# bcosm/CantorRL

Hardware: AMD Instinct MI355X
Metric: env-steps/sec (batched episodes) (higher is better)
Workload: dtype f64+f32; 1 GPU; configs[1]: 65,536 parallel envs/GPU, European call (BS rolling-ATM marks), GBM, v2 env, train_ppo_v2 reward; config_index=2, envs_per_gpu=65536, episode_length=252, mode=rollout, rollout_k=256, action_sets=1, parallelism=env-shard x1

## Files before the change

### cantorrl_amd/_lib.py

```python
import ctypes
import os

HERE = os.path.dirname(os.path.abspath(__file__))
LIB_PATH = os.environ.get("CANTORRL_HEDGEENV_LIB") or os.path.join(HERE, "lib", "libhedgeenv.so")

HE_ABI_VERSION = 4
HE_BOOK_MAX = 8
HE_OBS_DIM = 13
BOOK_TYPES = {"call": 0, "put": 1, "uo_call": 2}
HE_OK, HE_EINVAL, HE_ESHAPE, HE_EHIP, HE_ENOMEM, HE_ESTATE = range(6)
HE_MODE_REPLAY, HE_MODE_GBM, HE_MODE_HESTON = range(3)
HE_LOSS_MSE, HE_LOSS_ABS, HE_LOSS_CVAR, HE_LOSS_OTHER = range(4)
MODES = {"replay": HE_MODE_REPLAY, "gbm": HE_MODE_GBM, "heston": HE_MODE_HESTON}
HE_MARK_ROLLING_ATM, HE_MARK_FIXED_EUROPEAN = range(2)
MARKS = {"rolling_atm": HE_MARK_ROLLING_ATM, "fixed_european": HE_MARK_FIXED_EUROPEAN}


def loss_code(loss_type):
    return {"mse": HE_LOSS_MSE, "abs": HE_LOSS_ABS, "cvar": HE_LOSS_CVAR}.get(loss_type, HE_LOSS_OTHER)


class HeBookOption(ctypes.Structure):
    _fields_ = [
        ("type", ctypes.c_int32),
# ... 54 lines not shown
                            ("per_share_pnl_sum", "<f8"), ("reserved2", "<f8")])
assert EPISODE_RECORD.itemsize == 80

_P = ctypes.c_void_p
INFO_FIELDS = [
    ("step_pnl_total", "f8"), ("per_share_step_pnl", "f8"), ("raw_pnl_deviation_abs", "f8"),
    ("transaction_costs_total", "f8"), ("commission_cost", "f8"), ("slippage_cost", "f8"),
    ("reward_pnl_component", "f8"), ("transaction_cost_penalty", "f8"), ("theta_penalty", "f8"),
    ("reward_step", "f8"), ("portfolio_value", "f8"), ("cash", "f8"),
    ("call_contracts", "i4"), ("put_contracts", "i4"),
    ("scaled_float_call", "f4"), ("scaled_float_put", "f4"),
    ("requested_calls_rounded_clipped", "i4"), ("requested_puts_rounded_clipped", "i4"),
    ("actual_calls_traded", "i4"), ("actual_puts_traded", "i4"),
    ("initial_S0_for_episode", "f4"),
    ("current_stock_price", "f4"), ("current_volatility", "f4"),
    ("current_call_price", "f4"), ("current_put_price", "f4"), ("current_step", "i4"),
    ("current_episode_idx", "i4"),
]


class HeInfo(ctypes.Structure):
    _fields_ = [(name, _P) for name, _ in INFO_FIELDS]


EXPORTS = [
    "he_config_init", "he_create", "he_destroy", "he_last_error", "he_version", "he_load_paths",
    "he_seed", "he_reset", "he_reset_episodes", "he_step", "he_rollout", "he_num_envs", "he_episode_length",
    "he_num_episodes", "he_get_config", "he_state_size", "he_get_state", "he_set_state",
    "he_pcg64_seed_state", "he_host_episode_draws", "he_host_philox", "he_host_div_by", "he_host_div_byf", "he_time_next_step", "he_rollout_policy", "he_host_box_muller",
    "he_sync_market", "he_vecnorm_stats_len", "he_vecnorm_scratch_bytes", "he_vecnorm_init", "he_vecnorm_step",
    "he_vecnorm_apply", "he_vecnorm_attach", "he_vecnorm_attach_eval", "he_vecnorm_reset", "he_fixed_european_marks", "he_bs_delta_hedge", "he_count_nonfinite",
    "he_device_rng", "he_device_math", "he_host_math", "he_episode_summaries", "he_host_alloc", "he_host_free",
    "he_stream_wait", "he_step_signal", "he_signal_seq", "he_signal_wait", "he_host_episode_wrap",
    "he_host_vecnorm_sb3",
]


class HeVecnormParams(ctypes.Structure):
    _fields_ = [
        ("obs_dim", ctypes.c_int32),
        ("training", ctypes.c_int32),
        ("norm_obs", ctypes.c_int32),
        ("norm_reward", ctypes.c_int32),
        ("gamma", ctypes.c_double),
        ("clip_obs", ctypes.c_double),
        ("clip_reward", ctypes.c_double),
        ("epsilon", ctypes.c_double),
        ("moments", ctypes.c_int32),
        ("reserved", ctypes.c_int32 * 3),
    ]


HE_VN_MOMENTS_F64, HE_VN_MOMENTS_SB3 = range(2)
HE_VN_SB3_MAX_ENVS = 4096
VN_MOMENTS = {"f64": HE_VN_MOMENTS_F64, "sb3": HE_VN_MOMENTS_SB3}


class HeVecnormOut(ctypes.Structure):
    _fields_ = [(name, ctypes.c_void_p) for name in (
        "stats", "returns", "obs_out", "reward_out", "terminal_obs_out", "ep_return", "ep_length", "ep_return_done",
        "ep_length_done")]

_lib = None


class HedgeEnvError(RuntimeError):
    pass
# ... 26 lines not shown
        "he_step": (i32, [vp, vp, vp, vp, vp, vp, vp, ctypes.POINTER(HeInfo), vp]),
        "he_rollout": (i32, [vp, i32, vp, vp, vp, vp, vp]),
        "he_rollout_policy": (i32, [vp, i32, i32, vp, vp, vp, vp, vp, i64, vp, vp]),
        "he_num_envs": (i64, [vp]),
        "he_episode_length": (i32, [vp]),
        "he_num_episodes": (i64, [vp]),
        "he_get_config": (i32, [vp, ctypes.POINTER(HeConfig)]),
        "he_state_size": (ctypes.c_size_t, [vp]),
        "he_get_state": (i32, [vp, vp, ctypes.c_size_t]),
        "he_set_state": (i32, [vp, vp, ctypes.c_size_t]),
        "he_pcg64_seed_state": (i32, [u64, ctypes.POINTER(ctypes.c_uint64 * 4)]),
        "he_host_episode_draws": (i32, [u64, u64, i64, vp]),
        "he_host_philox": (i32, [u64, u64, u64, ctypes.POINTER(ctypes.c_uint32 * 4)]),
        "he_host_div_by": (i32, [ctypes.c_void_p, i64, ctypes.c_double, ctypes.c_void_p]),
        "he_host_div_byf": (i32, [ctypes.c_void_p, i64, ctypes.c_float, ctypes.c_void_p]),
        "he_host_box_muller": (i32, [ctypes.c_void_p, ctypes.c_void_p, i64, ctypes.c_void_p, ctypes.c_void_p]),
        "he_time_next_step": (i32, [vp, vp, vp]),
        "he_sync_market": (i32, [vp, vp]),
        "he_vecnorm_stats_len": (i64, [i32]),
        "he_vecnorm_scratch_bytes": (i64, [i64, i32]),
        "he_vecnorm_init": (i32, [vp, i32, vp]),
        "he_vecnorm_step": (i32, [ctypes.POINTER(HeVecnormParams), i64] + [vp] * 15 + [vp]),
        "he_vecnorm_apply": (i32, [ctypes.POINTER(HeVecnormParams), i64] + [vp] * 15 + [vp]),
        "he_vecnorm_attach": (i32, [vp, ctypes.POINTER(HeVecnormParams), vp, vp, vp]),
        "he_vecnorm_attach_eval": (i32, [vp, ctypes.POINTER(HeVecnormParams), ctypes.POINTER(HeVecnormOut)]),
        "he_vecnorm_reset": (i32, [ctypes.POINTER(HeVecnormParams), i64] + [vp] * 5 + [vp]),
        "he_host_vecnorm_sb3": (i32, [ctypes.POINTER(HeVecnormParams), i64] + [vp] * 9),
        "he_fixed_european_marks": (i32, [vp, i64, i32, ctypes.c_double, vp, vp, vp, vp]),
        "he_bs_delta_hedge": (i32, [vp, i64, i32, ctypes.c_double, ctypes.c_double, vp, vp]),
        "he_count_nonfinite": (i32, [vp, i64, vp, vp]),
        "he_device_rng": (i32, [u64, vp, vp, i64, vp, vp, vp]),
        "he_device_math": (i32, [i32, vp, i64, vp, vp]),
        "he_host_math": (i32, [i32, vp, i64, vp]),
        "he_host_episode_wrap": (i32, [vp, vp, vp, i64, i32, vp]),
        "he_episode_summaries": (i32, [vp, vp, vp]),
        "he_host_alloc": (i32, [ctypes.c_size_t, ctypes.POINTER(vp), ctypes.POINTER(vp)]),
        "he_host_free": (i32, [vp]),
        "he_stream_wait": (i32, [vp]),
        "he_step_signal": (i32, [vp, vp]),
        "he_signal_seq": (ctypes.c_uint32, [vp]),
        "he_signal_wait": (i32, [vp, vp, vp]),
    }
    ab = path != os.path.join(HERE, "lib", "libhedgeenv.so")
    for name, (res, args) in sig.items():
        if ab and not hasattr(lib, name):
            continue
        fn = getattr(lib, name)
        fn.restype = res
        fn.argtypes = args
    _lib = lib
    return lib


def check(lib, handle, status, what):
    if status != HE_OK:
        msg = lib.he_last_error(handle).decode() if handle else ""
        if status == HE_ESHAPE:
            raise ValueError(msg or "Data shapes are inconsistent.")
        raise HedgeEnvError(f"{what} failed (status {status}): {msg}")


def pcg64_seed_state(seed):
    lib = load()
    arr = (ctypes.c_uint64 * 4)()
    check(lib, None, lib.he_pcg64_seed_state(ctypes.c_uint64(seed), ctypes.byref(arr)), "he_pcg64_seed_state")
    return tuple(arr)
# ... 46 lines not shown
```

### cantorrl_amd/csrc/he_math.h

```cpp
#pragma once

#include <hip/hip_runtime.h>
#include <stdint.h>

#define HE_HD __host__ __device__ __forceinline__

namespace he {

HE_HD double fma_k(double a, double b, double c) {
#if defined(__HIP_DEVICE_COMPILE__)
    double r;
    asm("v_fma_f64 %0, %1, %2, %3" : "=v"(r) : "v"(a), "v"(b), "s"(c));
    return r;
#else
    return fma(a, b, c);
#endif
}

HE_HD double fma_kb(double a, double k, double c) {
#if defined(__HIP_DEVICE_COMPILE__)
    double r;
    asm("v_fma_f64 %0, %1, %2, %3" : "=v"(r) : "v"(a), "s"(k), "v"(c));
    return r;
#else
// ... 140 lines not shown
    return k <= T ? episode_wrap_le(t, k, T) : (t + k) % T;
}

struct u32x4 { uint32_t x, y, z, w; };

HE_HD uint32_t mulhi32(uint32_t a, uint32_t b) {
#if defined(__HIP_DEVICE_COMPILE__)
    return __umulhi(a, b);
#else
    return (uint32_t)(((uint64_t)a * (uint64_t)b) >> 32);
#endif
}

HE_HD u32x4 philox4x32_10(u32x4 c, uint32_t k0, uint32_t k1) {
    const uint32_t M0 = 0xD2511F53u, M1 = 0xCD9E8D57u;
    const uint32_t W0 = 0x9E3779B9u, W1 = 0xBB67AE85u;
#pragma unroll
    for (int r = 0; r < 10; ++r) {
        if (r) { k0 += W0; k1 += W1; }
        const uint64_t p0 = (uint64_t)M0 * c.x, p1 = (uint64_t)M1 * c.z;
        uint32_t hi0 = (uint32_t)(p0 >> 32), lo0 = (uint32_t)p0;
        uint32_t hi1 = (uint32_t)(p1 >> 32), lo1 = (uint32_t)p1;
        u32x4 o;
        o.x = hi1 ^ c.y ^ k0;
        o.y = lo1;
        o.z = hi0 ^ c.w ^ k1;
        o.w = lo0;
        c = o;
    }
    return c;
}

HE_HD double u01(uint32_t hi, uint32_t lo) {
    uint64_t k = ((((uint64_t)hi) << 32) | (uint64_t)lo) >> 12;
    return ((double)k + 0.5) * 2.220446049250313e-16;
}

HE_HD void sincos_2pi_u(double u2, double* sin_out, double* cos_out) {
    const double x = 4.0 * u2;
    const double q = rint(x);
    const double r = x - q;
    const double rr = r * r;
    double sp = 6.066935731106192e-12;
    sp = fma_k(sp, rr, -6.688035109811464e-10);
    sp = fma_k(sp, rr, 5.692172921967924e-08);
    sp = fma_k(sp, rr, -3.598843235212084e-06);
    sp = fma_k(sp, rr, 0.00016044118478735975);
    sp = fma_k(sp, rr, -0.004681754135318687);
    sp = fma_k(sp, rr, 0.07969262624616703);
    sp = fma_k(sp, rr, -0.6459640975062462);
    sp = fma_k(sp, rr, 1.5707963267948966);
    const double sn = r * sp;
    double cp = 6.565963114979468e-11;
    cp = fma_k(cp, rr, -6.386603083791849e-09);
    cp = fma_k(cp, rr, 4.710874778818169e-07);
    cp = fma_k(cp, rr, -2.5202042373060596e-05);
    cp = fma_k(cp, rr, 0.0009192602748394263);
    cp = fma_k(cp, rr, -0.020863480763352957);
    cp = fma_k(cp, rr, 0.253669507901048);
    cp = fma_k(cp, rr, -1.2337005501361697);
    const double cs = fma_k(cp, rr, 1.0);
    const int qi = (int)q & 3;
    const bool swp = (qi & 1) != 0;
    const double s_ = swp ? cs : sn, c_ = swp ? sn : cs;
    *sin_out = (qi & 2) ? -s_ : s_;
    *cos_out = ((qi + 1) & 2) ? -c_ : c_;
}

// ... 85 lines not shown
    p = fma_k(p, z, 0.005223977625442187842111847);
    p = fma_k(p, z, -0.02686617064513125175943235);
    p = fma_k(p, z, 0.1128379167095512573896159);
    p = fma_k(p, z, -0.376126389031837524632053);
    p = fma_k(p, z, 1.128379167095512573896159);
    return x * p;
}

HE_HD double ndtr(double a) {
    if (a != a) return a;
    const double SQRT1_2 = 0.70710678118654752440;
    double x = a * SQRT1_2;
    double z = fabs(x);
    double y;
    if (z < SQRT1_2) {
        y = 0.5 + 0.5 * erf_small(x);
    } else {
        y = 0.5 * erfc(z);
        if (x > 0) y = 1.0 - y;
    }
    return y;
}

HE_HD void ndtr_pair(double a, double* pos, double* neg) {
    if (a != a) {
        *pos = *neg = a;
        return;
    }
    const double SQRT1_2 = 0.70710678118654752440;
    double x = a * SQRT1_2;
    double z = fabs(x);
    if (z < SQRT1_2) {
        double e = (z < 0.25) ? erf_small4(x) : erf_small(x);
        *pos = 0.5 + 0.5 * e;
        *neg = 0.5 + 0.5 * (-e);
    } else {
        double y = 0.5 * erfc(z);
        if (x > 0) {
            *pos = 1.0 - y;
            *neg = y;
        } else {
            *pos = y;
            *neg = 1.0 - y;
        }
    }
}

HE_HD double norm_pdf(double x) {
    return exp(-(x * x) * 0.5) * 0.3989422804014327;
}

HE_HD double log_ratio(double S, double K) {
#if defined(__HIP_DEVICE_COMPILE__)
    double r = __builtin_amdgcn_rcp(K);
    r = fma(fma(-K, r, 1.0), r, r);
    r = fma(fma(-K, r, 1.0), r, r);
    const double y = (S - K) * r;
    if (!(fabs(y) < 0.0078125)) return log(S / K);
#else
    const double q = S / K;
    const double y = q - 1.0;
    if (!(fabs(y) < 0.0078125)) return log(q);
#endif
    double p = 1.0 / 9.0;
    p = fma_k(p, y, -1.0 / 8.0);
    p = fma_k(p, y, 1.0 / 7.0);
    p = fma_k(p, y, -1.0 / 6.0);
    p = fma_k(p, y, 1.0 / 5.0);
// ... 63 lines not shown
    for (int h = 0; h < NN; ++h) {
        const double xs = (fabs(x[h]) < 700.0) ? x[h] : 0.0;
        k[h] = rint(xs * 1.4426950408889634074);
        const double rh = fma_kb(-k[h], 6.93147180369123816490e-01, xs);
        r[h] = fma_kb(-k[h], 1.90821492927058770002e-10, rh);
        q[h] = 1.0 / 355687428096000.0;
    }
    constexpr double C[16] = {1.0 / 20922789888000.0, 1.0 / 1307674368000.0, 1.0 / 87178291200.0,
                              1.0 / 6227020800.0,     1.0 / 479001600.0,     1.0 / 39916800.0,
                              1.0 / 3628800.0,        1.0 / 362880.0,        1.0 / 40320.0,
                              1.0 / 5040.0,           1.0 / 720.0,           1.0 / 120.0,
                              1.0 / 24.0,             1.0 / 6.0,             0.5,
                              0.0};
#pragma unroll
    for (int c = 0; c < 15; ++c)
#pragma unroll
        for (int h = 0; h < NN; ++h) q[h] = fma_k(q[h], r[h], C[c]);
#pragma unroll
    for (int h = 0; h < NN; ++h) {
        const double s1 = 1.0 + r[h];
        const double e1 = (1.0 - s1) + r[h];
        out[h] = ldexp(s1 + fma(r[h] * r[h], q[h], e1), (int)k[h]);
    }
    bool big = false;
#pragma unroll
    for (int h = 0; h < NN; ++h) big = big || !(fabs(x[h]) < 700.0);
    if (he_any_lane(big)) {
#pragma unroll
        for (int h = 0; h < NN; ++h) out[h] = (fabs(x[h]) < 700.0) ? out[h] : exp(x[h]);
    }
}

template <int NN>
HE_HD void philox4x32_10_n(u32x4* c, uint32_t k0, uint32_t k1) {
    const uint32_t M0 = 0xD2511F53u, M1 = 0xCD9E8D57u;
    const uint32_t W0 = 0x9E3779B9u, W1 = 0xBB67AE85u;
#pragma unroll
    for (int rd = 0; rd < 10; ++rd) {
        if (rd) { k0 += W0; k1 += W1; }
#pragma unroll
        for (int h = 0; h < NN; ++h) {
            const uint64_t p0 = (uint64_t)M0 * c[h].x, p1 = (uint64_t)M1 * c[h].z;
            u32x4 o;
            o.x = (uint32_t)(p1 >> 32) ^ c[h].y ^ k0;
            o.y = (uint32_t)p1;
            o.z = (uint32_t)(p0 >> 32) ^ c[h].w ^ k1;
            o.w = (uint32_t)p0;
            c[h] = o;
        }
    }
}

template <int NN>
HE_HD void box_muller_n(const double* u1, const double* u2, double* z1, double* z2) {
    double s[NN], s2[NN], p[NN], ed[NN];
#pragma unroll
    for (int h = 0; h < NN; ++h) {
        int e;
        double m = frexp(u1[h], &e);
        const bool lo = m < 0.70710678118654752;
        m = lo ? m + m : m;
        ed[h] = (double)(lo ? e - 1 : e);
        s[h] = bm_quot(m);
        s2[h] = s[h] * s[h];
        p[h] = 1.0 / 19.0;
    }
// ... 41 lines not shown
        z1[h] = rad[h] * cosv;
        z2[h] = rad[h] * sinv;
    }
}

template <int NN>
HE_HD void ndtr_pair_n(const double* a, double* pos, double* neg) {
    const double SQRT1_2 = 0.70710678118654752440;
    double x[NN], z[NN], p[NN];
    bool easy = true;
#pragma unroll
    for (int h = 0; h < NN; ++h) {
        x[h] = a[h] * SQRT1_2;
        easy = easy && (fabs(x[h]) < 0.25);
        z[h] = x[h] * x[h];
        p[h] = 0.000001646211436588924740161296;
    }
    if (he_any_lane(!easy)) {
#pragma unroll
        for (int h = 0; h < NN; ++h) ndtr_pair(a[h], pos + h, neg + h);
        return;
    }
    constexpr double E[8] = {-0.00001492565035840625097746242, 0.0001205533298178966425102734,
                             -0.0008548327023450852832546658,  0.005223977625442187842111847,
                             -0.02686617064513125175943235,    0.1128379167095512573896159,
                             -0.376126389031837524632053,      1.128379167095512573896159};
#pragma unroll
    for (int c = 0; c < 8; ++c)
#pragma unroll
        for (int h = 0; h < NN; ++h) p[h] = fma_k(p[h], z[h], E[c]);
#pragma unroll
    for (int h = 0; h < NN; ++h) {
        const double e = x[h] * p[h];
        pos[h] = 0.5 + 0.5 * e;
        neg[h] = 0.5 + 0.5 * (-e);
    }
}

template <int NN>
HE_HD void log_ratio_n(const double* S, const double* K, double* out) {
    double y[NN], p[NN];
    bool easy = true;
#pragma unroll
    for (int h = 0; h < NN; ++h) {
#if defined(__HIP_DEVICE_COMPILE__)
        double r = __builtin_amdgcn_rcp(K[h]);
        r = fma(fma(-K[h], r, 1.0), r, r);
        r = fma(fma(-K[h], r, 1.0), r, r);
        y[h] = (S[h] - K[h]) * r;
#else
        const double q = S[h] / K[h];
        y[h] = q - 1.0;
#endif
        easy = easy && (fabs(y[h]) < 0.0078125);
        p[h] = 1.0 / 9.0;
    }
    if (he_any_lane(!easy)) {
#pragma unroll
        for (int h = 0; h < NN; ++h) out[h] = log_ratio(S[h], K[h]);
        return;
    }
    constexpr double L[8] = {-1.0 / 8.0, 1.0 / 7.0, -1.0 / 6.0, 1.0 / 5.0, -1.0 / 4.0, 1.0 / 3.0, -0.5, 1.0};
#pragma unroll
    for (int c = 0; c < 8; ++c)
#pragma unroll
        for (int h = 0; h < NN; ++h) p[h] = fma_k(p[h], y[h], L[c]);
#pragma unroll
    for (int h = 0; h < NN; ++h) out[h] = y[h] * p[h];
}

template <int NN>
HE_HD void bs_call_put_n(const double* S, const double* K, const BSConst& c, double* call, double* put) {
    if (c.intrinsic) {
#pragma unroll
        for (int h = 0; h < NN; ++h) bs_call_put(S[h], K[h], c, call + h, put + h);
        return;
    }
    double lr[NN], d[2 * NN], nd[2 * NN], md[2 * NN];
    log_ratio_n<NN>(S, K, lr);
#pragma unroll
    for (int h = 0; h < NN; ++h) {
        d[h] = (lr[h] + c.a) * c.inv_b;
        d[NN + h] = d[h] - c.b;
    }
    ndtr_pair_n<NN>(d, nd, md);
    ndtr_pair_n<NN>(d + NN, nd + NN, md + NN);
#pragma unroll
    for (int h = 0; h < NN; ++h) {
        const double Kd = K[h] * c.disc;
        const double cv = S[h] * nd[h] - Kd * nd[NN + h];
        const double pv = Kd * md[NN + h] - S[h] * md[h];
        call[h] = (cv < 0.0) ? 0.0 : cv;
        put[h] = (pv < 0.0) ? 0.0 : pv;
    }
}

struct Pcg64 {
    uint64_t sh, sl, ih, il;
    uint32_t has32, buf32;
};

HE_HD void pcg64_step(Pcg64& g) {
    const uint64_t MH = 0x2360ED051FC65DA4ull, ML = 0x4385DF649FCCF645ull;
#if defined(__HIP_DEVICE_COMPILE__)
    uint64_t lo = g.sl * ML;
    uint64_t hi = __umul64hi(g.sl, ML) + g.sl * MH + g.sh * ML;
#else
    unsigned __int128 p = (unsigned __int128)g.sl * ML;
    uint64_t lo = (uint64_t)p;
    uint64_t hi = (uint64_t)(p >> 64) + g.sl * MH + g.sh * ML;
#endif
    uint64_t nl = lo + g.il;
    uint64_t carry = nl < lo ? 1ull : 0ull;
    g.sl = nl;
    g.sh = hi + g.ih + carry;
}

HE_HD uint64_t pcg64_next64(Pcg64& g) {
    pcg64_step(g);
    uint64_t x = g.sh ^ g.sl;
    unsigned rot = (unsigned)(g.sh >> 58);
    return (x >> rot) | (x << ((64u - rot) & 63u));
}

HE_HD uint32_t pcg64_next32(Pcg64& g) {
    if (g.has32) {
// ... 50 lines not shown
```

### cantorrl_amd/csrc/hedge_env.hip

```cpp
#include <hip/hip_runtime.h>
#include <hip/hip_ext.h>

#include <math.h>
#include <stdarg.h>
#include <stdio.h>
#include <stdlib.h>
#include <string.h>

#include <chrono>
#include <new>
#include <type_traits>

#include "vn_moments.h"
#include <string>
#include <vector>

#include "../../include/hedge_env.h"
#include "he_math.h"

using namespace he;

namespace {

#define GLOBAL __attribute__((address_space(1)))
// ... 46 lines not shown
    double lnK, lnH, lnH2K;
    double invK;
    double invH;
};

struct Params {
    int64_t n;
    int64_t goff;
    int32_t T;
    int32_t variant, loss, record_metrics, autoreset, mode;
    int32_t tile_greeks;
    int32_t mt, maxh;
    float mt_f, maxh_f, T_f;
    float inv_maxh_f, inv_T_f;
    int32_t s0s_const;
    float s0s_f, inv_s0s_f;
    double s0s_d, inv_s0s_d;
    double inv_252;
    float init_cash_f;
    double tcpc, slip_frac, lam, w, theta, initial_cash;
    double shares_d, inv_shares;
    float shares_f;
    int32_t shares_zero;
    float r_f, tenor_f;
    double r_d, tenor_d, sqrt_tenor;
    int32_t tenor_small;
    uint32_t key0, key1;
    double s0;
    double var;
    float var_f;
    double sqrt_var, drift, sqrt_dt, mu, dt;
    BSConst bs;
    int32_t mark;
    double fe_K;
    float g_sigma, g_num_drift;
    double g_sst;
    double g_inv_sst;
    float g_sst_f, g_inv_sst_f;
    int32_t lds_tame;
    float sqrt_tenor_f;
    double h_kappa, h_theta, h_xi, h_rho, h_sqrt1mrho2;
    int32_t den_const;
    double den, inv_den;
    int32_t M;
    float4* tileA;
    float4* tileB;
    float rstv[4 + kObs];
    const float4* rec;
    const float4* recg;
    int64_t n_paths;
    int64_t rstride;
    int32_t roff;
    int32_t book_n;
    const BookOpt* book;
    const double* book_tab;
    int32_t book_rows;
    double bk_sig, bk_isig, bk_s2, bk_lam;
    double book_rst;
    double* tileC;
#ifdef HE_TIMING
    uint64_t* tim;
#endif
};

constexpr int32_t kRowOff = 7;
__host__ __device__ __forceinline__ int64_t replay_stride(int64_t T) { return ((T + 1 + kRowOff + 7) / 8) * 8; }
// ... 2189 lines not shown

            const int64_t gid = p.goff + pi;
            const uint64_t nf = a0 + (uint64_t)(kb + sl0);
            const uint32_t tpf = PLAIN ? 0u : episode_wrap(tpb, (uint32_t)sl0, T);
            double ex[kLdsH];
            double Vx[kLdsH];
            double Vin = Vbs;
            if constexpr (LOCK) {
                const uint64_t m0 = nf >> 1;
                const bool odd = (nf & 1) != 0;
                double zs[kLdsH];
                if (__ballot(odd) == 0ull) {
                    double zz[kLdsH];
                    philox_normals_n<kLdsH / 2>(p, gid, m0, zz);
#pragma unroll
                    for (int h = 0; h < kLdsH; ++h) zs[h] = zz[h];
                } else {
                    double zz[kLdsH + 2];
                    philox_normals_n<kLdsH / 2 + 1>(p, gid, m0, zz);
#pragma unroll
                    for (int h = 0; h < kLdsH; ++h) {
                        double a = zz[h], b = zz[h + 1];
                        asm volatile("" : "+v"(a), "+v"(b));
                        zs[h] = odd ? b : a;
                    }
                }
                double arg[kLdsH];
#pragma unroll
                for (int h = 0; h < kLdsH; ++h) {
                    Vx[h] = 0.0;
                    const double dW = p.sqrt_dt * zs[h];
                    arg[h] = p.drift + p.sqrt_var * dW;
                }
                exp_k_n<kLdsH>(arg, ex);
            } else if constexpr (!HESTON) {
                double zc = 0.0;
#pragma unroll
                for (int h = 0; h < kLdsH; ++h) {
                    ex[h] = 1.0;
                    Vx[h] = 0.0;
                    if (FULL || sl0 + h < len) {
                        const uint64_t n = nf + (uint64_t)h;
                        double z;
                        if (h == 0 || (n & 1) == 0) {
                            double z1, z2;
                            normals(p, gid, n >> 1, &z1, &z2);
                            z = (n & 1) ? z2 : z1;
                            zc = z2;
                        } else {
                            z = zc;
                        }
                        const double dW = p.sqrt_dt * z;
                        ex[h] = exp_k(p.drift + p.sqrt_var * dW);
                    }
                }
            } else {
                double w1[kLdsH], ws[kLdsH];
#pragma unroll
                for (int h = 0; h < kLdsH; ++h) w1[h] = ws[h] = 0.0;
#pragma unroll 1
                for (int h = 0; h < kLdsH; ++h) {
                    double a = 0.0, b = 0.0;
                    if (FULL || sl0 + h < len) {
                        double z1, z2;
                        normals(p, gid, nf + (uint64_t)h, &z1, &z2);
                        const double dw1 = p.sqrt_dt * z1, dw2 = p.sqrt_dt * z2;
                        a = dw1;
// ... 24 lines not shown
                    if (FULL || j < len) {
                        if (tq == 0) v = p.var;
                        vp = v < 0.0 ? 0.0 : v;
                        sq = sqrt(vp);
                        v = (v + p.h_kappa * (p.h_theta - vp) * p.dt) + p.h_xi * sq * w1all[j];
                        tq = (tq + 1 == T) ? 0u : tq + 1;
                    }
#pragma unroll
                    for (int h = 0; h < kLdsH; ++h) {
                        vpx[h] = (j == sl0 + h) ? vp : vpx[h];
                        sqx[h] = (j == sl0 + h) ? sq : sqx[h];
                        Vx[h] = (j == sl0 + h) ? v : Vx[h];
                    }
                }
                Vbs = v;
#pragma unroll
                for (int h = 0; h < kLdsH; ++h) {
                    const double drift = (p.mu - 0.5 * vpx[h]) * p.dt;
                    const double diff = sqx[h] * ws[h];
                    ex[h] = (FULL || sl0 + h < len) ? exp(drift + diff) : 1.0;
                }
            }
            double eall[kLdsM];
#pragma unroll
            for (int r = 0; r < kLdsLanes; ++r)
#pragma unroll
                for (int h = 0; h < kLdsH; ++h) eall[r * kLdsH + h] = __shfl(ex[h], (lane % kLdsPEnvs) + r * kLdsPEnvs);
            double Sx[kLdsH], Mx[kLdsH];
#pragma unroll
            for (int h = 0; h < kLdsH; ++h) Sx[h] = Sbs;
#pragma unroll
            for (int h = 0; h < kLdsH; ++h) Mx[h] = Mbs;
            double S = Sbs, Sin = Sbs, Mr = Mbs;
            if constexpr (kTame && FULL) {
                static_assert(!kTame || kLdsM == 2 * kLdsH, "two lanes per env");
                double Sa[kLdsM];
                uint32_t tp = tpb;
#pragma unroll
                for (int j = 0; j < kLdsM; ++j) {
                    if (!PLAIN && tp == 0) S = p.s0;
                    const double Sn = S * eall[j];
                    S = (Sn < 1e-8) ? 1e-8 : Sn;
                    if (!PLAIN) tp = (tp + 1 == T) ? 0u : tp + 1;
                    Sa[j] = S;
                }
                const bool hi = sub != 0;
#pragma unroll
                for (int h = 0; h < kLdsH; ++h) Sx[h] = hi ? Sa[kLdsH + h] : Sa[h];
                Sin = hi ? Sa[kLdsH - 1] : Sbs;
            } else {
                uint32_t tp = tpb;
#pragma unroll
                for (int j = 0; j < kLdsM; ++j) {
                    if (j == sl0) Sin = S;
                    if (FULL || j < len) {
                        if (!PLAIN && tp == 0) {
                            S = p.s0;
                            if (BOOK) Mr = p.s0;
                        }
                        const double Sn = S * eall[j];
                        S = (Sn < 1e-8) ? 1e-8 : Sn;
                        if (BOOK) Mr = np_max(Mr, S);
                        if (!PLAIN) tp = (tp + 1 == T) ? 0u : tp + 1;
                    }
#pragma unroll
                    for (int h = 0; h < kLdsH; ++h) Sx[h] = (j == sl0 + h) ? S : Sx[h];
                    if (BOOK) {
#pragma unroll
                        for (int h = 0; h < kLdsH; ++h) Mx[h] = (j == sl0 + h) ? Mr : Mx[h];
                    }
                }
            }
            Sbs = S;
            if (BOOK) Mbs = Mr;
            uint32_t tp = tpf;
            const int wb = bp % LdsMarketT<MODE, BOOK, LEAN>::NB;
            double lkC[kLdsH], lkP[kLdsH];
            if constexpr (LOCK) {
                double Sm[kLdsH], Km[kLdsH];
                uint32_t tq = tpf;
#pragma unroll
                for (int h = 0; h < kLdsH; ++h) {
                    if constexpr (PLAIN) {
                        Sm[h] = Sx[h];
                    } else {
                        const bool last = tq + 1 == T;
                        const double Sprev = (h == 0) ? Sin : Sx[h - 1];
                        Sm[h] = last ? ((tq == 0) ? p.s0 : Sprev) : Sx[h];
                        tq = (tq + 1 == T) ? 0u : tq + 1;
                    }
                    Km[h] = rint(Sm[h]);
                }
                bs_call_put_n<kLdsH>(Sm, Km, p.bs, lkC, lkP);
            }
            if constexpr (kTame) {
                uint32_t verdict = 0u;
                if constexpr (LOCK && PLAIN) {
                    uint32_t smin = (uint32_t)__double2hiint(Sx[0]), smax = smin;
                    uint32_t mmin = (uint32_t)__double2hiint(lkC[0]), mmax = mmin;
#pragma unroll
                    for (int h = 0; h < kLdsH; ++h) {
                        const uint32_t sh = (uint32_t)__double2hiint(Sx[h]);
                        const uint32_t ch = (uint32_t)__double2hiint(lkC[h]), ph = (uint32_t)__double2hiint(lkP[h]);
                        smin = sh < smin ? sh : smin;
                        smax = sh > smax ? sh : smax;
                        mmin = ch < mmin ? ch : mmin;
                        mmax = ch > mmax ? ch : mmax;
                        mmin = ph < mmin ? ph : mmin;
                        mmax = ph > mmax ? ph : mmax;
                    }
                    const bool ok = smin >= 0x40500000u && smax < 0x41600000u && mmin >= 0x38100000u && mmax < 0x47e00000u;
                    verdict = __ballot(!ok) == 0ull ? 0xffffffffu : 0u;
                }
                W.tame[wb][pw] = verdict;
            }
            if constexpr (LOCK) {
#pragma unroll
                for (int h = 0; h < kLdsH; ++h) {
                    const int sl = sl0 + h;
                    W.sc[wb][sl][le] = make_float2((float)Sx[h], (float)lkC[h]);
                    W.pp[wb][sl][le] = (float)lkP[h];
                }
            } else {
                double rS[kLdsH], rV[kLdsH];
#pragma unroll
                for (int h = 0; h < kLdsH; ++h) {
                    rS[h] = Sx[h];
                    rV[h] = HESTON ? Vx[h] : p.var;
                }
                double Sprev = Sin, Vprev = Vin;
#pragma unroll 1
                for (int h = 0; h < kLdsH; ++h) {
                    if (FULL || sl0 + h < len) {
                        const bool last = tp + 1 == T;
                        const double Sm = last ? ((tp == 0) ? p.s0 : Sprev) : rS[0];
                        const double Vh = rV[0];
                        const double Vm = HESTON ? (last ? ((tp == 0) ? p.var : Vprev) : Vh) : p.var;
                        float C, P;
                        marks<MODE, !LEAN>(p, Sm, Vm, last ? tp : tp + 1u, &C, &P);
                        const int sl = sl0 + h;
                        W.sc[wb][sl][le] = make_float2((float)rS[0], C);
                        W.pp[wb][sl][le] = P;
                        if (HESTON) W.vv[HESTON ? wb : 0][HESTON ? sl : 0][le] = (float)Vh;
                        tp = (tp + 1 == T) ? 0u : tp + 1;
                    }
// ... 625 lines not shown
    const u32x4 x = philox4x32_10(c, k0, k1);
    if (words) {
        words[4 * k] = x.x;
        words[4 * k + 1] = x.y;
        words[4 * k + 2] = x.z;
        words[4 * k + 3] = x.w;
    }
    if (normals) box_muller(u01(x.x, x.y), u01(x.z, x.w), normals + 2 * k, normals + 2 * k + 1);
}

HE_HD void math_group(int32_t op, const double* x, int64_t count, double* out, int64_t g, const BSConst& bs) {
    const double pad = (op == 4 || op == 5) ? 0.5 : ((op == 2 || op == 3) ? 500.0 : 0.0);
    double a[4], r[4], q[4];
    for (int h = 0; h < 4; ++h) a[h] = (4 * g + h < count) ? x[4 * g + h] : pad;
    switch (op) {
        case 0:
            for (int h = 0; h < 4; ++h) r[h] = exp_k(a[h]);
            break;
        case 1:
            exp_k_n<4>(a, r);
            break;
        case 2:
            for (int h = 0; h < 4; ++h) bs_call_put(a[h], rint(a[h]), bs, r + h, q + h);
            break;
        case 3: {
            double K[4];
            for (int h = 0; h < 4; ++h) K[h] = rint(a[h]);
            bs_call_put_n<4>(a, K, bs, r, q);
            break;
        }
        case 4:
            box_muller(a[0], a[1], r, r + 1);
            box_muller(a[2], a[3], r + 2, r + 3);
            break;
        default: {
            const double u1[2] = {a[0], a[2]}, u2[2] = {a[1], a[3]};
            double z1[2], z2[2];
            box_muller_n<2>(u1, u2, z1, z2);
            r[0] = z1[0], r[1] = z2[0], r[2] = z1[1], r[3] = z2[1];
        }
    }
    for (int h = 0; h < 4; ++h)
        if (4 * g + h < count) out[4 * g + h] = r[h];
}

__global__ void device_math_kernel(int32_t op, const double* x, int64_t count, double* out, BSConst bs) {
    const int64_t g = (int64_t)blockIdx.x * blockDim.x + threadIdx.x;
    if (4 * g >= count) return;
    math_group(op, x, count, out, g, bs);
}

static BSConst default_bs() {
    BSConst c;
    const double sig = sqrt(0.029028), T = 30.0 / 252.0, r = 0.04;
    c.intrinsic = 0;
    c.a = (r + 0.5 * pow(sig, 2.0)) * T;
    c.b = sig * sqrt(T);
    c.inv_b = 1.0 / c.b;
    c.disc = exp(-r * T);
    return c;
}

template <int MODE>
__global__ __launch_bounds__(kBlock) void reset_kernel(Params p, State s, Market cur, const int64_t* ids,
                                                       int64_t count, float* obs, he_info inf, const int64_t* eps) {
    const int64_t j = (int64_t)blockIdx.x * kBlock + threadIdx.x;
// ... 242 lines not shown
    p.tenor_f = (float)c.option_tenor_years;
    p.r_d = c.risk_free_rate;
    p.tenor_d = c.option_tenor_years;
    p.sqrt_tenor = sqrt(c.option_tenor_years);
    p.tenor_small = c.option_tenor_years <= 1e-6;
    p.key0 = (uint32_t)(c.seed & 0xFFFFFFFFu);
    p.key1 = (uint32_t)(c.seed >> 32);
    p.s0 = c.s0;
    p.var = c.variance;
    p.var_f = (float)c.variance;
    p.mu = c.mu;
    p.dt = c.dt;
    p.sqrt_dt = sqrt(c.dt);
    p.drift = (c.mu - 0.5 * c.variance) * c.dt;
    p.sqrt_var = sqrt(c.variance < 0.0 ? 0.0 : c.variance);
    double sig = sqrt(c.variance < 0.0 ? 0.0 : c.variance);
    double T = c.option_tenor_years, r = c.risk_free_rate;
    p.bs.intrinsic = (T <= 0.0) || (sig <= 0.0);
    p.bs.a = (r + 0.5 * pow(sig, 2.0)) * T;
    p.bs.b = sig * sqrt(T);
    p.bs.inv_b = 1.0 / p.bs.b;
    p.bs.disc = exp(-r * T);
    p.mark = c.mark;
    p.fe_K = rint(c.s0);
    float vf = (float)c.variance;
    float vmax = (vf != vf) ? vf : (vf > 1e-8f ? vf : 1e-8f);
    p.g_sigma = sqrtf(vmax);
    p.g_num_drift = ((float)r + 0.5f * powf(p.g_sigma, 2.0f)) * (float)T;
    p.g_sst = (double)p.g_sigma * sqrt(T);
    p.g_inv_sst = 1.0 / p.g_sst;
    p.g_sst_f = (float)p.g_sst;
    p.g_inv_sst_f = (float)p.g_inv_sst;
    p.lds_tame = lds_tame_handle(p) ? 1 : 0;
    p.sqrt_tenor_f = (float)p.sqrt_tenor;
    p.h_kappa = c.heston_kappa;
    p.h_theta = c.heston_theta;
    p.h_xi = c.heston_xi;
    p.h_rho = c.heston_rho;
    double omr = 1.0 - c.heston_rho * c.heston_rho;
    p.h_sqrt1mrho2 = sqrt(omr < 0.0 ? 0.0 : omr);
    p.T = c.episode_length;
    p.T_f = (float)c.episode_length;
    p.inv_maxh_f = 1.0f / p.maxh_f;
    p.inv_T_f = 1.0f / p.T_f;
    p.inv_252 = 1.0 / 252.0;
    p.M = c.market_block;
    p.tileA = p.tileB = nullptr;
    memcpy(p.rstv, env->rstv, sizeof(p.rstv));
    if (is_generate(env)) {
        float s0 = p.rstv[0];
        bool small = s0 < 1e-6f;
        float f = small ? 25.0f : (s0 > 25.0f || s0 != s0 ? s0 : 25.0f);
        if (c.loss_type == HE_LOSS_MSE) p.den = small ? (625.0 + 1e-9) : (double)(f * f + 1e-9f);
        else p.den = small ? (25.0 + 1e-9) : (double)(f + 1e-9f);
        p.inv_den = 1.0 / p.den;
        p.den_const = 1;
        p.s0s_const = 1;
        p.s0s_f = f;
        p.inv_s0s_f = 1.0f / f;
        p.s0s_d = (double)f;
        p.inv_s0s_d = 1.0 / (double)f;
    }
    p.rec = env->rec;
    p.recg = env->recg;
    p.book_n = is_generate(env) ? c.book_size : 0;
    p.bk_sig = sqrt(p.var < 0.0 ? 0.0 : p.var);
// ... 677 lines not shown
he_status he_debug_lds_timing(void* host, size_t bytes) {
    const size_t cap = sizeof(g_lds_tim);
    if (bytes > cap) bytes = cap;
    return hipMemcpyFromSymbol(host, HIP_SYMBOL(g_lds_tim), bytes, 0, hipMemcpyDeviceToHost) == hipSuccess ? HE_OK : HE_EHIP;
}
#endif

#ifdef HE_LDS_HWID
he_status he_debug_lds_hwid(void* host, size_t bytes) {
    const size_t cap = sizeof(g_lds_hwid);
    if (bytes > cap) bytes = cap;
    return hipMemcpyFromSymbol(host, HIP_SYMBOL(g_lds_hwid), bytes, 0, hipMemcpyDeviceToHost) == hipSuccess ? HE_OK : HE_EHIP;
}
#endif

#ifdef HE_TIMING
he_status he_debug_timing(void* host, size_t bytes) {
    const size_t cap = (size_t)5 * 8192 * 2 * 8;
    if (bytes > cap) bytes = cap;
    return hipMemcpy(host, g_tim, bytes, hipMemcpyDeviceToHost) == hipSuccess ? HE_OK : HE_EHIP;
}
#endif

he_status he_device_rng(uint64_t seed, const uint64_t* env_ids, const uint64_t* step_index, int64_t count,
                        uint32_t* words, double* normals, void* stream) {
    if (count < 0 || (count > 0 && (!env_ids || !step_index))) return HE_EINVAL;
    if (count == 0) return HE_OK;
    hipLaunchKernelGGL(device_rng_kernel, dim3((unsigned)((count + 255) / 256)), dim3(256), 0, (hipStream_t)stream,
                       (uint32_t)seed, (uint32_t)(seed >> 32), env_ids, step_index, count, words, normals);
    return hipGetLastError() == hipSuccess ? HE_OK : HE_EHIP;
}

he_status he_device_math(int32_t op, const double* x, int64_t count, double* out, void* stream) {
    if (op < 0 || op > 5 || count < 0 || (count > 0 && (!x || !out))) return HE_EINVAL;
    if (count == 0) return HE_OK;
    const int64_t groups = (count + 3) / 4;
    hipLaunchKernelGGL(device_math_kernel, dim3((unsigned)((groups + 255) / 256)), dim3(256), 0, (hipStream_t)stream,
                       op, x, count, out, default_bs());
    return hipGetLastError() == hipSuccess ? HE_OK : HE_EHIP;
}

he_status he_host_math(int32_t op, const double* x, int64_t count, double* out) {
    if (op < 0 || op > 5 || count < 0 || (count > 0 && (!x || !out))) return HE_EINVAL;
    const BSConst bs = default_bs();
    for (int64_t g = 0; 4 * g < count; ++g) math_group(op, x, count, out, g, bs);
    return HE_OK;
}

he_status he_host_episode_wrap(const uint32_t* t, const uint32_t* k, const uint32_t* T, int64_t count, int32_t le,
                               uint32_t* out) {
    if (count < 0 || ((!t || !k || !T || !out) && count > 0)) return HE_EINVAL;
    for (int64_t j = 0; j < count; ++j)
        out[j] = le ? episode_wrap_le(t[j], k[j], T[j]) : episode_wrap(t[j], k[j], T[j]);
    return HE_OK;
}

he_status he_host_div_by(const double* a, int64_t count, double b, double* out) {
    if ((!a || !out) && count > 0) return HE_EINVAL;
    const double y = 1.0 / b;
    for (int64_t k = 0; k < count; ++k) out[k] = div_by(a[k], b, y);
    return HE_OK;
}

he_status he_host_box_muller(const double* u1, const double* u2, int64_t count, double* z1, double* z2) {
    if ((!u1 || !u2 || !z1 || !z2) && count > 0) return HE_EINVAL;
    for (int64_t k = 0; k < count; ++k) box_muller(u1[k], u2[k], z1 + k, z2 + k);
    return HE_OK;
}

he_status he_host_div_byf(const float* a, int64_t count, float b, float* out) {
    if ((!a || !out) && count > 0) return HE_EINVAL;
    const float y = 1.0f / b;
    for (int64_t k = 0; k < count; ++k) out[k] = div_byf(a[k], b, y);
    return HE_OK;
}

he_status he_seed(he_env* env, const int64_t* env_ids, const uint64_t* seeds, int64_t count) {
    if (!env) return HE_EINVAL;
    if (!seeds || count < 1) return fail(env, HE_EINVAL, "he_seed needs >= 1 seed");
    DeviceGuard dg(env->cfg.device);
    const int64_t N = env->cfg.n_envs;
    HE_HIP(env, hipDeviceSynchronize());
    if (env->cfg.mode == HE_MODE_REPLAY) {
        std::vector<uint64_t> pcg((size_t)(4 * N));
        std::vector<uint32_t> pcgb((size_t)(2 * N));
        HE_HIP(env, hipMemcpy(pcg.data(), env->s.pcg, pcg.size() * 8, hipMemcpyDeviceToHost));
        HE_HIP(env, hipMemcpy(pcgb.data(), env->s.pcgb, pcgb.size() * 4, hipMemcpyDeviceToHost));
        for (int64_t k = 0; k < count; ++k) {
            int64_t i = env_ids ? env_ids[k] : k;
            if (i < 0 || i >= N) return fail(env, HE_EINVAL, "env id %lld out of range", (long long)i);
            uint64_t st[4];
            seed_sequence_pcg64(seeds[k], st);
            for (int w = 0; w < 4; ++w) pcg[(size_t)(w * N + i)] = st[w];
            pcgb[(size_t)i] = 0;
// ... 449 lines not shown
```

### include/hedge_env.h

```cpp
#ifndef HEDGE_ENV_H
#define HEDGE_ENV_H

#include <stddef.h>
#include <stdint.h>

#ifdef __cplusplus
extern "C" {
#endif

#define HE_ABI_VERSION 4
#define HE_BOOK_MAX 8
#define HE_OBS_DIM 13
#define HE_ACT_DIM 2

typedef enum he_status {
    HE_OK = 0,
    HE_EINVAL = 1,
    HE_ESHAPE = 2,
    HE_EHIP = 3,
    HE_ENOMEM = 4,
    HE_ESTATE = 5
} he_status;

typedef enum he_mode {
// ... 147 lines not shown
he_status he_rollout_policy(he_env* env, int32_t k_steps, int32_t policy, float* actions_out, float* obs,
                            float* reward, uint8_t* terminated, he_episode_record* records,
                            int64_t record_capacity, unsigned long long* record_count, void* stream);

he_status he_episode_summaries(he_env* env, float* out, void* stream);

he_status he_sync_market(he_env* env, void* stream);

he_status he_time_next_step(he_env* env, void* start_event, void* stop_event);

he_status he_host_alloc(size_t bytes, void** host_ptr, void** device_ptr);
he_status he_host_free(void* host_ptr);
he_status he_stream_wait(void* stream);

he_status he_step_signal(he_env* env, uint32_t* flag);
uint32_t he_signal_seq(const he_env* env);
he_status he_signal_wait(he_env* env, const uint32_t* flag_host, void* stream);

int64_t he_num_envs(const he_env* env);
int32_t he_episode_length(const he_env* env);
int64_t he_num_episodes(const he_env* env);
he_status he_get_config(const he_env* env, he_config* out);

size_t he_state_size(const he_env* env);
he_status he_get_state(he_env* env, void* host_buf, size_t size);
he_status he_set_state(he_env* env, const void* host_buf, size_t size);

he_status he_pcg64_seed_state(uint64_t seed, uint64_t state[4]);

he_status he_host_episode_draws(uint64_t seed, uint64_t n_paths, int64_t count, int64_t* out);
he_status he_host_philox(uint64_t seed, uint64_t env_id, uint64_t n, uint32_t out[4]);
he_status he_host_div_by(const double* a, int64_t count, double b, double* out);
he_status he_host_box_muller(const double* u1, const double* u2, int64_t count, double* z1, double* z2);
he_status he_host_div_byf(const float* a, int64_t count, float b, float* out);
he_status he_host_episode_wrap(const uint32_t* t, const uint32_t* k, const uint32_t* T, int64_t count, int32_t le,
                               uint32_t* out);
he_status he_device_rng(uint64_t seed, const uint64_t* env_ids, const uint64_t* step_index, int64_t count,
                        uint32_t* words, double* normals, void* stream);
he_status he_device_math(int32_t op, const double* x, int64_t count, double* out, void* stream);
he_status he_host_math(int32_t op, const double* x, int64_t count, double* out);

#define HE_VN_MOMENTS_F64 0
#define HE_VN_MOMENTS_SB3 1
#define HE_VN_SB3_MAX_ENVS 4096
typedef struct he_vecnorm_params {
    int32_t obs_dim;
    int32_t training;
    int32_t norm_obs;
    int32_t norm_reward;
    double gamma;
    double clip_obs;
    double clip_reward;
    double epsilon;
    int32_t moments;
    int32_t reserved[3];
} he_vecnorm_params;

int64_t he_vecnorm_stats_len(int32_t obs_dim);
int64_t he_vecnorm_scratch_bytes(int64_t n, int32_t obs_dim);

he_status he_vecnorm_init(double* stats, int32_t obs_dim, void* stream);

he_status he_vecnorm_step(const he_vecnorm_params* p, int64_t n, const float* obs, const float* reward,
                          const uint8_t* done, const float* terminal_obs, double* returns, double* stats,
                          void* scratch, float* obs_out, float* reward_out, float* terminal_obs_out,
                          double* ep_return, int32_t* ep_length, double* ep_return_done,
// ... 43 lines not shown
```

Before: 65.50 billion env-steps/s.

## Add small-argument exp path, bit-cast u01, and skip clamps when paths are tame

Uses a range-bounded Taylor exp for GBM increments when drift and volatility are provably small. It also converts uniforms through a mantissa bit-cast instead of an int-to-double conversion, and fuses the normal-CDF affine steps into FMAs. In the plain tame path it first runs an unclamped price recurrence with a wave-level check, falling back to the clamped loop only when some lane is out of range. Option-price flooring is deferred the same way. These cut per-step ALU work in the hot rollout kernel, at the cost of more code paths that rely on the bound and ballot checks for correctness.

```diff
diff --git a/cantorrl_amd/_lib.py b/cantorrl_amd/_lib.py
--- a/cantorrl_amd/_lib.py
+++ b/cantorrl_amd/_lib.py
@@ -110,7 +110,7 @@
     "he_vecnorm_apply", "he_vecnorm_attach", "he_vecnorm_attach_eval", "he_vecnorm_reset", "he_fixed_european_marks", "he_bs_delta_hedge", "he_count_nonfinite",
     "he_device_rng", "he_device_math", "he_host_math", "he_episode_summaries", "he_host_alloc", "he_host_free",
     "he_stream_wait", "he_step_signal", "he_signal_seq", "he_signal_wait", "he_host_episode_wrap",
-    "he_host_vecnorm_sb3",
+    "he_host_vecnorm_sb3", "he_host_u01", "he_host_exp_small",
 ]
 
 
@@ -203,6 +203,8 @@
         "he_device_rng": (i32, [u64, vp, vp, i64, vp, vp, vp]),
         "he_device_math": (i32, [i32, vp, i64, vp, vp]),
         "he_host_math": (i32, [i32, vp, i64, vp]),
+        "he_host_u01": (i32, [vp, vp, i64, vp]),
+        "he_host_exp_small": (i32, [ctypes.c_double, ctypes.c_double, ctypes.c_double]),
         "he_host_episode_wrap": (i32, [vp, vp, vp, i64, i32, vp]),
         "he_episode_summaries": (i32, [vp, vp, vp]),
         "he_host_alloc": (i32, [ctypes.c_size_t, ctypes.POINTER(vp), ctypes.POINTER(vp)]),
diff --git a/cantorrl_amd/csrc/he_math.h b/cantorrl_amd/csrc/he_math.h
--- a/cantorrl_amd/csrc/he_math.h
+++ b/cantorrl_amd/csrc/he_math.h
@@ -196,8 +196,9 @@
 }
 
 HE_HD double u01(uint32_t hi, uint32_t lo) {
-    uint64_t k = ((((uint64_t)hi) << 32) | (uint64_t)lo) >> 12;
-    return ((double)k + 0.5) * 2.220446049250313e-16;
+    const uint64_t k = ((((uint64_t)hi) << 32) | (uint64_t)lo) >> 12;
+    const double w = __builtin_bit_cast(double, 0x3FF0000000000000ull | k);
+    return (w - 1.0) + 1.1102230246251565e-16;
 }
 
 HE_HD void sincos_2pi_u(double u2, double* sin_out, double* cos_out) {
@@ -349,8 +350,8 @@
     double z = fabs(x);
     if (z < SQRT1_2) {
         double e = (z < 0.25) ? erf_small4(x) : erf_small(x);
-        *pos = 0.5 + 0.5 * e;
-        *neg = 0.5 + 0.5 * (-e);
+        *pos = fma(0.5, e, 0.5);
+        *neg = fma(-0.5, e, 0.5);
     } else {
         double y = 0.5 * erfc(z);
         if (x > 0) {
@@ -480,6 +481,34 @@
 }
 
 template <int NN>
+HE_HD void exp_small_n(const double* x, double* out) {
+    double q[NN];
+#pragma unroll
+    for (int h = 0; h < NN; ++h) q[h] = 1.0 / 355687428096000.0;
+    constexpr double C[16] = {1.0 / 20922789888000.0, 1.0 / 1307674368000.0, 1.0 / 87178291200.0,
+                              1.0 / 6227020800.0,     1.0 / 479001600.0,     1.0 / 39916800.0,
+                              1.0 / 3628800.0,        1.0 / 362880.0,        1.0 / 40320.0,
+                              1.0 / 5040.0,           1.0 / 720.0,           1.0 / 120.0,
+                              1.0 / 24.0,             1.0 / 6.0,             0.5,
+                              0.0};
+#pragma unroll
+    for (int c = 0; c < 15; ++c)
+#pragma unroll
+        for (int h = 0; h < NN; ++h) q[h] = fma_k(q[h], x[h], C[c]);
+#pragma unroll
+    for (int h = 0; h < NN; ++h) {
+        const double s1 = 1.0 + x[h];
+        const double e1 = (1.0 - s1) + x[h];
+        out[h] = s1 + fma(x[h] * x[h], q[h], e1);
+    }
+}
+
+HE_HD bool exp_small_bound(double drift, double sqrt_var, double sqrt_dt) {
+    const double b = (fabs(drift) + fabs(sqrt_var) * fabs(sqrt_dt) * 8.6) * 1.4426950408889634;
+    return b < 0.49;
+}
+
+template <int NN>
 HE_HD void philox4x32_10_n(u32x4* c, uint32_t k0, uint32_t k1) {
     const uint32_t M0 = 0xD2511F53u, M1 = 0xCD9E8D57u;
     const uint32_t W0 = 0x9E3779B9u, W1 = 0xBB67AE85u;
@@ -587,8 +616,8 @@
 #pragma unroll
     for (int h = 0; h < NN; ++h) {
         const double e = x[h] * p[h];
-        pos[h] = 0.5 + 0.5 * e;
-        neg[h] = 0.5 + 0.5 * (-e);
+        pos[h] = fma(0.5, e, 0.5);
+        neg[h] = fma(-0.5, e, 0.5);
     }
 }
 
@@ -624,7 +653,7 @@
     for (int h = 0; h < NN; ++h) out[h] = y[h] * p[h];
 }
 
-template <int NN>
+template <int NN, bool FLOOR = true>
 HE_HD void bs_call_put_n(const double* S, const double* K, const BSConst& c, double* call, double* put) {
     if (c.intrinsic) {
 #pragma unroll
@@ -645,8 +674,8 @@
         const double Kd = K[h] * c.disc;
         const double cv = S[h] * nd[h] - Kd * nd[NN + h];
         const double pv = Kd * md[NN + h] - S[h] * md[h];
-        call[h] = (cv < 0.0) ? 0.0 : cv;
-        put[h] = (pv < 0.0) ? 0.0 : pv;
+        call[h] = (FLOOR && cv < 0.0) ? 0.0 : cv;
+        put[h] = (FLOOR && pv < 0.0) ? 0.0 : pv;
     }
 }
 
diff --git a/cantorrl_amd/csrc/hedge_env.hip b/cantorrl_amd/csrc/hedge_env.hip
--- a/cantorrl_amd/csrc/hedge_env.hip
+++ b/cantorrl_amd/csrc/hedge_env.hip
@@ -102,6 +102,7 @@
     double sqrt_var, drift, sqrt_dt, mu, dt;
     BSConst bs;
     int32_t mark;
+    int32_t lds_exp_small;
     double fe_K;
     float g_sigma, g_num_drift;
     double g_sst;
@@ -2357,7 +2358,8 @@
                     const double dW = p.sqrt_dt * zs[h];
                     arg[h] = p.drift + p.sqrt_var * dW;
                 }
-                exp_k_n<kLdsH>(arg, ex);
+                if (p.lds_exp_small) exp_small_n<kLdsH>(arg, ex);
+                else exp_k_n<kLdsH>(arg, ex);
             } else if constexpr (!HESTON) {
                 double zc = 0.0;
 #pragma unroll
@@ -2448,22 +2450,48 @@
 #pragma unroll
             for (int h = 0; h < kLdsH; ++h) Mx[h] = Mbs;
             double S = Sbs, Sin = Sbs, Mr = Mbs;
+            bool s_tame = false;
             if constexpr (kTame && FULL) {
                 static_assert(!kTame || kLdsM == 2 * kLdsH, "two lanes per env");
                 double Sa[kLdsM];
-                uint32_t tp = tpb;
-#pragma unroll
-                for (int j = 0; j < kLdsM; ++j) {
-                    if (!PLAIN && tp == 0) S = p.s0;
-                    const double Sn = S * eall[j];
-                    S = (Sn < 1e-8) ? 1e-8 : Sn;
-                    if (!PLAIN) tp = (tp + 1 == T) ? 0u : tp + 1;
-                    Sa[j] = S;
+                const bool hi = sub != 0;
+                auto own = [&]() {
+#pragma unroll
+                    for (int h = 0; h < kLdsH; ++h) Sx[h] = hi ? Sa[kLdsH + h] : Sa[h];
+                    Sin = hi ? Sa[kLdsH - 1] : Sbs;
+                };
+                bool clamped = !PLAIN;
+                if constexpr (PLAIN) {
+#pragma unroll
+                    for (int j = 0; j < kLdsM; ++j) {
+                        S = S * eall[j];
+                        Sa[j] = S;
+                    }
+                    own();
+                    uint32_t smin = 0xffffffffu, smax = 0u;
+#pragma unroll
+                    for (int h = 0; h < kLdsH; ++h) {
+                        const uint32_t sh = (uint32_t)__double2hiint(Sx[h]);
+                        smin = sh < smin ? sh : smin;
+                        smax = sh > smax ? sh : smax;
+                    }
+                    s_tame = __ballot(!(smin >= 0x40500000u && smax < 0x41600000u)) == 0ull;
+                    clamped = !s_tame;
                 }
-                const bool hi = sub != 0;
-#pragma unroll
-                for (int h = 0; h < kLdsH; ++h) Sx[h] = hi ? Sa[kLdsH + h] : Sa[h];
-                Sin = hi ? Sa[kLdsH - 1] : Sbs;
+                if (clamped) {
+                    if constexpr (PLAIN) asm volatile("");
+                    S = Sbs;
+                    uint32_t tp = tpb;
+#pragma unroll
+                    for (int j = 0; j < kLdsM; ++j) {
+                        if (!PLAIN && tp == 0) S = p.s0;
+                        const double Sn = S * eall[j];
+                        S = (Sn < 1e-8) ? 1e-8 : Sn;
+                        if (!PLAIN) tp = (tp + 1 == T) ? 0u : tp + 1;
+                        Sa[j] = S;
+                    }
+                    own();
+                }
             } else {
                 uint32_t tp = tpb;
 #pragma unroll
@@ -2507,26 +2535,30 @@
                     }
                     Km[h] = rint(Sm[h]);
                 }
-                bs_call_put_n<kLdsH>(Sm, Km, p.bs, lkC, lkP);
+                bs_call_put_n<kLdsH, !(kTame && PLAIN)>(Sm, Km, p.bs, lkC, lkP);
             }
             if constexpr (kTame) {
                 uint32_t verdict = 0u;
                 if constexpr (LOCK && PLAIN) {
-                    uint32_t smin = (uint32_t)__double2hiint(Sx[0]), smax = smin;
                     uint32_t mmin = (uint32_t)__double2hiint(lkC[0]), mmax = mmin;
 #pragma unroll
                     for (int h = 0; h < kLdsH; ++h) {
-                        const uint32_t sh = (uint32_t)__double2hiint(Sx[h]);
                         const uint32_t ch = (uint32_t)__double2hiint(lkC[h]), ph = (uint32_t)__double2hiint(lkP[h]);
-                        smin = sh < smin ? sh : smin;
-                        smax = sh > smax ? sh : smax;
                         mmin = ch < mmin ? ch : mmin;
                         mmax = ch > mmax ? ch : mmax;
                         mmin = ph < mmin ? ph : mmin;
                         mmax = ph > mmax ? ph : mmax;
                     }
-                    const bool ok = smin >= 0x40500000u && smax < 0x41600000u && mmin >= 0x38100000u && mmax < 0x47e00000u;
-                    verdict = __ballot(!ok) == 0ull ? 0xffffffffu : 0u;
+                    const bool m_tame = __ballot(!(mmin >= 0x38100000u && mmax < 0x47e00000u)) == 0ull;
+                    if (!m_tame) {
+                        asm volatile("");
+#pragma unroll
+                        for (int h = 0; h < kLdsH; ++h) {
+                            lkC[h] = (lkC[h] < 0.0) ? 0.0 : lkC[h];
+                            lkP[h] = (lkP[h] < 0.0) ? 0.0 : lkP[h];
+                        }
+                    }
+                    verdict = (s_tame && m_tame) ? 0xffffffffu : 0u;
                 }
                 W.tame[wb][pw] = verdict;
             }
@@ -3218,6 +3250,9 @@
         case 4:
             box_muller(a[0], a[1], r, r + 1);
             box_muller(a[2], a[3], r + 2, r + 3);
+            break;
+        case 6:
+            exp_small_n<4>(a, r);
             break;
         default: {
             const double u1[2] = {a[0], a[2]}, u2[2] = {a[1], a[3]};
@@ -3526,6 +3561,7 @@
     p.g_sst_f = (float)p.g_sst;
     p.g_inv_sst_f = (float)p.g_inv_sst;
     p.lds_tame = lds_tame_handle(p) ? 1 : 0;
+    p.lds_exp_small = exp_small_bound(p.drift, p.sqrt_var, p.sqrt_dt) ? 1 : 0;
     p.sqrt_tenor_f = (float)p.sqrt_tenor;
     p.h_kappa = c.heston_kappa;
     p.h_theta = c.heston_theta;
@@ -4269,7 +4305,7 @@
 }
 
 he_status he_device_math(int32_t op, const double* x, int64_t count, double* out, void* stream) {
-    if (op < 0 || op > 5 || count < 0 || (count > 0 && (!x || !out))) return HE_EINVAL;
+    if (op < 0 || op > 6 || count < 0 || (count > 0 && (!x || !out))) return HE_EINVAL;
     if (count == 0) return HE_OK;
     const int64_t groups = (count + 3) / 4;
     hipLaunchKernelGGL(device_math_kernel, dim3((unsigned)((groups + 255) / 256)), dim3(256), 0, (hipStream_t)stream,
@@ -4278,7 +4314,7 @@
 }
 
 he_status he_host_math(int32_t op, const double* x, int64_t count, double* out) {
-    if (op < 0 || op > 5 || count < 0 || (count > 0 && (!x || !out))) return HE_EINVAL;
+    if (op < 0 || op > 6 || count < 0 || (count > 0 && (!x || !out))) return HE_EINVAL;
     const BSConst bs = default_bs();
     for (int64_t g = 0; 4 * g < count; ++g) math_group(op, x, count, out, g, bs);
     return HE_OK;
@@ -4297,6 +4333,18 @@
     const double y = 1.0 / b;
     for (int64_t k = 0; k < count; ++k) out[k] = div_by(a[k], b, y);
     return HE_OK;
+}
+
+he_status he_host_u01(const uint32_t* hi, const uint32_t* lo, int64_t count, double* out) {
+    if ((!hi || !lo || !out) && count > 0) return HE_EINVAL;
+    for (int64_t k = 0; k < count; ++k) out[k] = u01(hi[k], lo[k]);
+    return HE_OK;
+}
+
+int32_t he_host_exp_small(double mu, double variance, double dt) {
+    const double drift = (mu - 0.5 * variance) * dt;
+    const double sqrt_var = sqrt(variance < 0.0 ? 0.0 : variance);
+    return exp_small_bound(drift, sqrt_var, sqrt(dt)) ? 1 : 0;
 }
 
 he_status he_host_box_muller(const double* u1, const double* u2, int64_t count, double* z1, double* z2) {
diff --git a/include/hedge_env.h b/include/hedge_env.h
--- a/include/hedge_env.h
+++ b/include/hedge_env.h
@@ -203,6 +203,8 @@
 he_status he_host_philox(uint64_t seed, uint64_t env_id, uint64_t n, uint32_t out[4]);
 he_status he_host_div_by(const double* a, int64_t count, double b, double* out);
 he_status he_host_box_muller(const double* u1, const double* u2, int64_t count, double* z1, double* z2);
+he_status he_host_u01(const uint32_t* hi, const uint32_t* lo, int64_t count, double* out);
+int32_t he_host_exp_small(double mu, double variance, double dt);
 he_status he_host_div_byf(const float* a, int64_t count, float b, float* out);
 he_status he_host_episode_wrap(const uint32_t* t, const uint32_t* k, const uint32_t* T, int64_t count, int32_t le,
                                uint32_t* out);
```

Measured after the change: 66.43 billion env-steps/s (median of 6 runs). No clear change (+1.4%).
